# kubewharf/kubebrain

Measured on AMD Instinct MI355X. Metric: range+txn ops/s (90/10, Range limit=500) + watch events/s, higher is better.
Workload: dtype u8

## Files before the change

### kubebrain_amd/__init__.py

```python
from __future__ import annotations

import ctypes
import os

_HERE = os.path.dirname(os.path.abspath(__file__))
LIB_PATH = os.path.join(_HERE, "libkbslab.so")


def build(force: bool = False) -> str:
    import subprocess

    src_dir = os.path.join(_HERE, "csrc")
    srcs = [os.path.join(src_dir, f) for f in ("slab.hip", "store.cc", "cabi.cc",
                                               "comm.cc", "slab_dev.h", "store.h",
                                               "wpoll.h", "lplan.h", "gplan.h",
                                               "stepstage.h", "dmerge.h", "cplan.h")]
    srcs.append(os.path.join(_HERE, "..", "include", "kb_slab.h"))
    stale = force or not os.path.exists(LIB_PATH) or any(
        os.path.getmtime(s) > os.path.getmtime(LIB_PATH) for s in srcs)
    if stale:
        subprocess.check_call(["make", "-C", src_dir])
    return LIB_PATH


def load_library() -> ctypes.CDLL:
    if not os.path.exists(LIB_PATH):
        build()
    return ctypes.CDLL(LIB_PATH)


def open_store(store_prefix: bytes = b"/registry", **kw):
    from .client import Store

    if not os.path.exists(LIB_PATH):
        build()
    try:
        return Store(LIB_PATH, "kb_", store_prefix=store_prefix, **kw)
    except RuntimeError as e:
        lib = ctypes.CDLL(LIB_PATH)
        buf = ctypes.create_string_buffer(512)
        code = lib.kb_last_error(buf, 512)
        raise RuntimeError(
            f"kubebrain_amd: kb_new failed (status {code}): "
            f"{buf.value.decode(errors='replace')}") from e
```

### kubebrain_amd/csrc/slab.hip

```cpp

#include <hip/hip_runtime.h>

#include <chrono>
#include <cstdio>
#include <cstring>

#include "cplan.h"
#include "dmerge.h"
#include "slab_dev.h"
#include "stepstage.h"

namespace kbslab {

#define HIP_CHECK(expr)                                                    \
  do {                                                                     \
    hipError_t _e = (expr);                                                \
    if (_e != hipSuccess) {                                                \
      if (err) *err = std::string(#expr) + ": " + hipGetErrorString(_e);   \
      return false;                                                        \
    }                                                                      \
  } while (0)

#define HIP_CHECK_NULL(expr)                                               \
  do {                                                                     \
    hipError_t _e = (expr);                                                \
    if (_e != hipSuccess) {                                                \
      if (err) *err = std::string(#expr) + ": " + hipGetErrorString(_e);   \
      return nullptr;                                                      \
    }                                                                      \
  } while (0)

static inline int64_t ceil_div(int64_t a, int64_t b) { return (a + b - 1) / b; }


__device__ __forceinline__ int keycmp96(const uint8_t* a, const uint8_t* b) {
  const uint64_t* A = (const uint64_t*)a;
  const uint64_t* B = (const uint64_t*)b;
#pragma unroll
  for (int i = 0; i < KEYW / 8; ++i) {
    uint64_t x = A[i], y = B[i];
    if (x != y) {
      x = __builtin_bswap64(x);
      y = __builtin_bswap64(y);
      return x < y ? -1 : 1;
    }
  }
  return 0;
}

__device__ __forceinline__ int keycmp_ext(
    const uint8_t* a96, uint32_t alen, uint64_t ako, const uint8_t* aspill,
    const uint8_t* b96, uint32_t blen, uint64_t bko, const uint8_t* bspill) {
  int c = keycmp96(a96, b96);
  if (c || (alen <= (uint32_t)KEYW && blen <= (uint32_t)KEYW)) return c;
  uint32_t at = alen > (uint32_t)KEYW ? alen - KEYW : 0;
  uint32_t bt = blen > (uint32_t)KEYW ? blen - KEYW : 0;
  const uint8_t* ap = aspill + ako;
  const uint8_t* bp = bspill + bko;
  uint32_t m = at < bt ? at : bt;
  for (uint32_t i = 0; i < m; ++i)
    if (ap[i] != bp[i]) return ap[i] < bp[i] ? -1 : 1;
  return at == bt ? 0 : (at < bt ? -1 : 1);
}

struct Run {
  const uint8_t* keys;
  const uint64_t* meta;
  const uint64_t* rev;
  const uint64_t* vo;
  const uint64_t* ko;
};

struct QKey {
  const uint8_t* k96;
  uint32_t len;
  uint64_t ko;
  const uint8_t* tails;
};

__device__ __forceinline__ QKey row_qk(const Run& r, const uint8_t* spill,
                                       int64_t i) {
  return QKey{r.keys + i * KEYW, meta_klen(r.meta[i]), r.ko[i], spill};
}

__device__ __forceinline__ int rowcmp_q(const Run& r, const uint8_t* spill,
                                        int64_t i, const QKey& q) {
  return keycmp_ext(r.keys + i * KEYW, meta_klen(r.meta[i]), r.ko[i], spill,
                    q.k96, q.len, q.ko, q.tails);
}

__device__ int64_t d_lb_range(const Run& r, const uint8_t* spill, int64_t lo,
                              int64_t hi, const QKey& q, uint64_t qrev) {
  while (lo < hi) {
    int64_t mid = (lo + hi) >> 1;
    int c = rowcmp_q(r, spill, mid, q);
    if (c < 0 || (c == 0 && r.rev[mid] < qrev)) lo = mid + 1; else hi = mid;
  }
  return lo;
}

__device__ int64_t d_lb_wave(const Run& r, const uint8_t* spill, int64_t n,
                             const QKey& q, uint64_t qrev) {
  const int lane = threadIdx.x & 63;
  int64_t lo = 0, hi = n;
  while (hi - lo > 64) {
    int64_t step = (hi - lo) >> 6;
    int64_t p = lo + (int64_t)(lane + 1) * step;
    bool lt = false;
    if (p < hi) {
      int c = rowcmp_q(r, spill, p, q);
      lt = c < 0 || (c == 0 && r.rev[p] < qrev);
    }
    int k = __popcll(__ballot(lt));
    int64_t nlo = lo + (int64_t)k * step;
    int64_t nhi = k == 64 ? hi : min(lo + (int64_t)(k + 1) * step, hi);
    lo = nlo;
    hi = nhi;
  }
  int64_t p = lo + lane;
  bool ge = false;
  if (p < hi) {
    int c = rowcmp_q(r, spill, p, q);
    ge = !(c < 0 || (c == 0 && r.rev[p] < qrev));
  }
  uint64_t b = __ballot(ge);
  return b ? lo + (__ffsll((unsigned long long)b) - 1) : hi;
}

template <typename T>
__device__ __forceinline__ T block_excl_scan(T v, T* wsum, T* total) {
  const int lane = threadIdx.x & 63, w = threadIdx.x >> 6;
  const int nw = blockDim.x >> 6;
  T inc = v;
#pragma unroll
  for (int off = 1; off < 64; off <<= 1) {
    T o = __shfl_up(inc, off);
    if (lane >= off) inc += o;
  }
  if (lane == 63) wsum[w] = inc;
  __syncthreads();
  T base = 0, tot = 0;
  for (int i = 0; i < nw; ++i) {
    T s = wsum[i];
    if (i < w) base += s;
    tot += s;
  }
  __syncthreads();
  *total = tot;
  return base + inc - v;
}

__device__ __forceinline__ bool rows_same_key(const uint8_t* keys,
                                              const uint64_t* meta,
                                              const uint64_t* ko,
                                              const uint8_t* spill, int64_t i,
                                              int64_t j) {
  const uint64_t* a = (const uint64_t*)(keys + i * KEYW);
  const uint64_t* b = (const uint64_t*)(keys + j * KEYW);
#pragma unroll
  for (int k = 0; k < KEYW / 8; ++k)
    if (a[k] != b[k]) return false;
  uint32_t al = meta_klen(meta[i]), bl = meta_klen(meta[j]);
  if (al <= (uint32_t)KEYW && bl <= (uint32_t)KEYW) return true;
  if (al != bl) return false;
  const uint8_t* ap = spill + ko[i];
  const uint8_t* bp = spill + ko[j];
  for (uint32_t t = 0; t < al - (uint32_t)KEYW; ++t)
    if (ap[t] != bp[t]) return false;
  return true;
}

__global__ void k_same_next(const uint8_t* __restrict__ keys,
                            uint64_t* __restrict__ meta,
                            const uint64_t* __restrict__ ko,
                            const uint8_t* __restrict__ spill, int64_t n) {
  int64_t i = (int64_t)blockIdx.x * blockDim.x + threadIdx.x;
  if (i >= n) return;
// ... 90 lines not shown
        uint64_t sh = shadow ? shadow[i] : UINT64_MAX;
        if (rv > 0 && rv <= R && !(m & M_TOMB) &&
            !(sh != UINT64_MAX && sh <= R))
          win = !(m & M_SAME_NEXT) || rvn > R;
      }
      if (win) flags |= 1ull << r;
    }
    if (dbg0) { unsigned long long t1 = wall_clock64(); atomicAdd(&dbg[1], t1 - tprev); tprev = t1; }
    uint32_t wcnt = 0;
    for (int r = 0; r < rounds; ++r)
      wcnt += (uint32_t)__popcll(__ballot((flags >> r) & 1));
    if (dbg0) { unsigned long long t2 = wall_clock64(); atomicAdd(&dbg[2], t2 - tprev); tprev = t2; }
    if (lane == 0) wave_cnt[w] = (int)wcnt;
    __syncthreads();
    int64_t waveoff = 0, tile_total = 0;
    for (int k = 0; k < NW; ++k) {
      if (k < w) waveoff += wave_cnt[k];
      tile_total += wave_cnt[k];
    }
    if (out && wcnt) {
      uint32_t done = 0;
      for (int r = 0; r < rounds; ++r) {
        uint64_t b = __ballot((flags >> r) & 1);
        if ((flags >> r) & 1) {
          int64_t idx = cnt + waveoff + done +
                        (int64_t)__popcll(b & ((1ull << lane) - 1));
          if (idx < cap && idx < out_cap)
            out[idx] = (uint64_t)(wbase + ((int64_t)r << 6) + lane) | tagbit;
        }
        done += (uint32_t)__popcll(b);
      }
    }
    if (dbg0) { unsigned long long t3 = wall_clock64(); atomicAdd(&dbg[3], t3 - tprev); tprev = t3; }
    cnt += tile_total;
    scanned += min(TILE, hi - t);
    if (cnt >= cap) break;
    __syncthreads();
  }
  *total_out = cnt;
  if (scanned_accum) *scanned_accum += scanned;
  int64_t written = cnt < cap ? cnt : cap;
  if (written > out_cap) written = out_cap;
  return out ? written : 0;
}

__device__ int64_t d_lb_winlist(const uint64_t* rows, int64_t n, const Run& b,
                                const Run& d, const uint8_t* spill,
                                const QKey& q) {
  int64_t lo = 0, hi = n;
  while (lo < hi) {
    int64_t mid = (lo + hi) >> 1;
    uint64_t rt = rows[mid];
    const Run& rr = (rt & ROW_TAG_DELTA) ? d : b;
    if (rowcmp_q(rr, spill, (int64_t)(rt & ROW_MASK), q) < 0) lo = mid + 1;
    else hi = mid;
  }
  return lo;
}

__global__ void k_range_bounds(Run b, int64_t n, Run d, int64_t dn,
                               const uint8_t* __restrict__ spill,
                               const uint8_t* __restrict__ qtails,
                               const DevRangeQ* __restrict__ qs, int nq,
                               int64_t* __restrict__ bounds_g ,
                               unsigned long long* __restrict__ counters) {
  int q = blockIdx.x;
  if (q >= nq) return;
  if (q == 0 && threadIdx.x == 0) { counters[0] = 0; counters[1] = 0; }
  const DevRangeQ& Q = qs[q];
  const QKey qstart{Q.start, Q.start_klen, Q.start_ko, qtails};
  const QKey qend{Q.end, Q.end_klen, Q.end_ko, qtails};
  int w = threadIdx.x >> 6;
  int64_t r = -1;
  if (w == 0) r = d_lb_wave(b, spill, n, qstart, Q.start_rev);
  else if (w == 1) r = d_lb_wave(b, spill, n, qend, 0);
  else if (w == 2) r = d_lb_wave(d, spill, dn, qstart, Q.start_rev);
  else if (w == 3) r = d_lb_wave(d, spill, dn, qend, 0);
  if (w < 4 && (threadIdx.x & 63) == 0) bounds_g[(int64_t)q * 4 + w] = r;
}

__global__ void k_range_scan2(
    Run b, int64_t n, Run d, int64_t dn, const uint8_t* __restrict__ spill,
    const uint8_t* __restrict__ qtails, const DevRangeQ* __restrict__ qs,
    int nq, int64_t max_cap,
    uint64_t* __restrict__ rows_b, uint64_t* __restrict__ rows_d,
    uint64_t* __restrict__ rows_m, int64_t* __restrict__ found_out,
    int64_t* __restrict__ total_out, unsigned long long* __restrict__ scanned_out,
    const int64_t* __restrict__ bounds_g,
    const uint64_t* __restrict__ shadow,
    unsigned long long* dbg) {
  int q = blockIdx.x;
  if (q >= nq) return;
  __shared__ int wave_cnt[SCAN_T_MAX / 64];
  const DevRangeQ& Q = qs[q];
  const bool dbg0 = dbg && threadIdx.x == 0;
  unsigned long long tk0 = dbg0 ? wall_clock64() : 0;
  const int64_t lo_s = bounds_g[(int64_t)q * 4 + 0];
  const int64_t hi_s = bounds_g[(int64_t)q * 4 + 1];
  const int64_t dlo_s = bounds_g[(int64_t)q * 4 + 2];
  const int64_t dhi_s = bounds_g[(int64_t)q * 4 + 3];
  if (dbg0) { unsigned long long tkb = wall_clock64(); atomicAdd(&dbg[0], tkb - tk0); }
  const int64_t cap = Q.cap > 0 ? Q.cap : INT64_MAX;
  int64_t scanned = 0;
  int64_t dtotal = 0, btotal = 0;
  uint64_t* outd = Q.count_only ? nullptr : rows_d + (int64_t)q * max_cap;
  uint64_t* outb = Q.count_only ? nullptr : rows_b + (int64_t)q * max_cap;
  int64_t nB = scan_run_winners(d, spill, dlo_s, dhi_s, Q.read_rev,
                                cap, outd, max_cap, ROW_TAG_DELTA, nullptr,
                                &dtotal, &scanned, wave_cnt, dbg);
  __syncthreads();
  int64_t nA = scan_run_winners(b, spill, lo_s, hi_s, Q.read_rev, cap,
                                outb, max_cap, 0, dn ? shadow : nullptr,
                                &btotal, &scanned, wave_cnt, dbg);
  __syncthreads();
  unsigned long long tkm = dbg0 ? wall_clock64() : 0;
  int64_t cap_m = nA + nB;
  if (cap_m > cap) cap_m = cap;
  if (cap_m > max_cap) cap_m = max_cap;
  if (!Q.count_only) {
    uint64_t* outm = rows_m + (int64_t)q * max_cap;
    for (int64_t j = threadIdx.x; j < nA + nB; j += blockDim.x) {
      uint64_t rt;
      int64_t pos;
      if (j < nA) {
        rt = outb[j];
        QKey k = row_qk(b, spill, (int64_t)(rt & ROW_MASK));
        pos = j + d_lb_winlist(outd, nB, b, d, spill, k);
      } else {
        rt = outd[j - nA];
        QKey k = row_qk(d, spill, (int64_t)(rt & ROW_MASK));
        pos = (j - nA) + d_lb_winlist(outb, nA, b, d, spill, k);
      }
      if (pos < cap_m) outm[pos] = rt;
    }
  }
  if (dbg0) {
    unsigned long long tke = wall_clock64();
    atomicAdd(&dbg[4], tke - tkm);
    atomicAdd(&dbg[5], tke - tk0);
    atomicMax(&dbg[6], tke - tk0);
    atomicAdd(&dbg[7], 1ull);
  }
  if (threadIdx.x == 0) {
    total_out[q] = btotal + dtotal;
    found_out[q] = Q.count_only ? 0 : cap_m;
    atomicAdd(scanned_out, (unsigned long long)scanned);
  }
}

__global__ void k_get2(Run b, Run d, int64_t n, int64_t dn,
                       const uint8_t* __restrict__ spill,
                       const uint8_t* __restrict__ qtails,
                       const uint8_t* __restrict__ heap,
                       const DevGetQ* __restrict__ qs, int nq, int copy_vals,
                       uint8_t* __restrict__ out, int64_t slot,
                       uint64_t* __restrict__ orev, uint64_t* __restrict__ ometa,
                       int32_t* __restrict__ ofound, int32_t* __restrict__ oovf) {
  int q = blockIdx.x * (blockDim.x / 64) + (threadIdx.x >> 6);
  int lane = threadIdx.x & 63;
  if (q >= nq) return;
  const DevGetQ& Q = qs[q];
  const QKey qk{Q.key, Q.klen, Q.ko, qtails};
  int64_t row = -1;
  int isdelta = 0;
  uint64_t nr = Q.read_rev == UINT64_MAX ? UINT64_MAX : Q.read_rev + 1;
  if (dn > 0) {
    int64_t ub = d_lb_wave(d, spill, dn, qk, nr);
    if (ub > 0) {
      int64_t c = ub - 1;
      if (d.rev[c] >= 1 && rowcmp_q(d, spill, c, qk) == 0) {
        row = c;
        isdelta = 1;
      }
    }
  }
  if (row < 0) {
    int64_t ub = d_lb_wave(b, spill, n, qk, nr);
    if (ub > 0) {
      int64_t c = ub - 1;
      if (b.rev[c] >= 1 && rowcmp_q(b, spill, c, qk) == 0) row = c;
    }
  }
  if (row < 0) {
    if (lane == 0) { ofound[q] = 0; oovf[q] = 0; }
    return;
  }
  const uint64_t* meta = isdelta ? d.meta : b.meta;
  const uint64_t* rev = isdelta ? d.rev : b.rev;
  const uint64_t* vo = isdelta ? d.vo : b.vo;
  uint64_t m = meta[row];
  uint32_t vlen = meta_vlen(m);
  if (lane == 0) {
    ofound[q] = 1;
    orev[q] = rev[row];
    ometa[q] = m;
    oovf[q] = (copy_vals && vlen > slot) ? 1 : 0;
  }
  if (!copy_vals || vlen > slot) return;
  const uint8_t* vs = heap + vo[row];
  uint8_t* vd = out + (int64_t)q * slot;
  uint32_t w16 = vlen >> 4;
  for (uint32_t b = lane; b < w16; b += 64)
    ((uint4*)vd)[b] = ((const uint4*)vs)[b];
  if (lane == 0)
    for (uint32_t b = w16 * 16; b < vlen; ++b) vd[b] = vs[b];
}

__device__ __forceinline__ int64_t rec_bytes(uint32_t klen, uint32_t vlen) {
  return 16 + ((klen + 15) & ~15u) + ((vlen + 15) & ~15u);
}

__global__ void k_gather(Run b, Run d,
                         const uint8_t* __restrict__ heap,
                         const uint64_t* __restrict__ rows_out, int64_t max_cap,
                         const int64_t* __restrict__ found_out,
                         const DevRangeQ* __restrict__ qs, int nq,
                         uint8_t* __restrict__ gbuf, int64_t qcap,
                         int64_t* __restrict__ offs,
                         int64_t* __restrict__ gbytes_out,
                         int32_t* __restrict__ overflow,
                         unsigned long long* __restrict__ bytes_out) {
  int q = blockIdx.x;
  if (q >= nq) return;
  int64_t nwin = found_out[q];
  const bool konly = qs[q].keys_only != 0;
  const uint64_t* rows = rows_out + (int64_t)q * max_cap;
  int64_t* qoffs = offs + (int64_t)q * max_cap;
  __shared__ int64_t lds[256];
  __shared__ int64_t base_s;
  if (threadIdx.x == 0) base_s = 0;
  __syncthreads();
  for (int64_t c0 = 0; c0 < nwin; c0 += blockDim.x) {
    int64_t j = c0 + threadIdx.x;
// ... 253 lines not shown
                       const int32_t* __restrict__ overflow,
                       uint8_t* __restrict__ out, int nq) {
  int q = blockIdx.x;
  if (q >= nq) return;
  if (overflow[q]) return;
  int64_t bytes = gbytes[q];
  const uint4* src = (const uint4*)(gbuf + (int64_t)q * qcap);
  uint4* dst = (uint4*)(out + goffs[q]);
  int64_t words = bytes / 16;
  for (int64_t w = threadIdx.x; w < words; w += blockDim.x) dst[w] = src[w];
}

__global__ void k_block_scan(const uint64_t* __restrict__ in,
                             uint64_t* __restrict__ out,
                             uint64_t* __restrict__ sums, int64_t n) {
  __shared__ uint64_t lds[256];
  int64_t base = (int64_t)blockIdx.x * 256;
  int t = threadIdx.x;
  uint64_t v = base + t < n ? in[base + t] : 0;
  lds[t] = v;
  __syncthreads();
  for (int off = 1; off < 256; off <<= 1) {
    uint64_t add = t >= off ? lds[t - off] : 0;
    __syncthreads();
    lds[t] += add;
    __syncthreads();
  }
  if (base + t < n) out[base + t] = lds[t] - v;
  if (t == 255) sums[blockIdx.x] = lds[255];
}

__global__ void k_add_offsets(uint64_t* __restrict__ out,
                              const uint64_t* __restrict__ block_offs, int64_t n) {
  int64_t i = (int64_t)blockIdx.x * 256 + threadIdx.x;
  if (i < n) out[i] += block_offs[blockIdx.x];
}

__global__ void k_merge_newn(const uint64_t* __restrict__ dropx, int64_t n,
                             int64_t m, int64_t* __restrict__ out_n) {
  if (threadIdx.x == 0 && blockIdx.x == 0) *out_n = n - (int64_t)dropx[n] + m;
}

__global__ void k_fill_u64(uint64_t* a, uint64_t v, int64_t n) {
  int64_t i = (int64_t)blockIdx.x * blockDim.x + threadIdx.x;
  if (i < n) a[i] = v;
}

__global__ void k_find_bounds(Run a, int64_t n, const uint8_t* spill,
                              const uint8_t* bkeys, const uint64_t* brevs, int nb,
                              int64_t* out) {
  int i = blockIdx.x * blockDim.x + threadIdx.x;
  if (i < nb)
    out[i] = d_lb_range(a, spill, 0, n,
                        QKey{bkeys + (int64_t)i * KEYW, (uint32_t)KEYW, 0, nullptr},
                        brevs[i]);
}

__global__ void k_compact_mark(const uint64_t* __restrict__ meta,
                               const uint64_t* __restrict__ rev,
                               const uint64_t* __restrict__ vo, int64_t lo,
                               int64_t hi, uint64_t compact_rev,
                               uint64_t timeout_rev, uint64_t* __restrict__ keep) {
  int64_t i = lo + (int64_t)blockIdx.x * blockDim.x + threadIdx.x;
  if (i >= hi) return;
  uint64_t r = rev[i], m = meta[i];
  if (timeout_rev != 0 && (m & M_EVENTS)) {
    if (r == 0) {
      if (vo[i] <= timeout_rev) { keep[i] = 0; return; }
    } else if (r <= timeout_rev) { keep[i] = 0; return; }
  }
  if (r > compact_rev) return;
  if (r == 0) {
    if ((m & M_FLAG9) && vo[i] <= compact_rev) keep[i] = 0;
    return;
  }
  if (m & M_TOMB) { keep[i] = 0; return; }
  if ((m & M_SAME_NEXT) && rev[i + 1] <= compact_rev) keep[i] = 0;
}

__global__ void k_heap_sizes(const uint64_t* __restrict__ keep,
                             const uint64_t* __restrict__ rev,
                             const uint64_t* __restrict__ meta,
                             uint64_t* __restrict__ sz, int64_t n) {
  int64_t i = (int64_t)blockIdx.x * blockDim.x + threadIdx.x;
  if (i >= n) return;
  sz[i] = (keep[i] && rev[i] > 0) ? ((meta_vlen(meta[i]) + 15) & ~15ull) : 0;
}

__global__ void k_compact_scatter(const uint8_t* __restrict__ keysA,
                                  const uint64_t* __restrict__ metaA,
                                  const uint64_t* __restrict__ revA,
                                  const uint64_t* __restrict__ voA,
                                  const uint64_t* __restrict__ koA,
                                  const uint64_t* __restrict__ keep,
                                  const uint64_t* __restrict__ nidx,
                                  const uint64_t* __restrict__ heap_off,
                                  const uint64_t* __restrict__ spill_off,
                                  uint8_t* __restrict__ keysB,
                                  uint64_t* __restrict__ metaB,
                                  uint64_t* __restrict__ revB,
                                  uint64_t* __restrict__ voB,
                                  uint64_t* __restrict__ koB, int64_t n) {
  int64_t i = (int64_t)blockIdx.x * blockDim.x + threadIdx.x;
  if (i >= n || !keep[i]) return;
  int64_t j = (int64_t)nidx[i];
  revB[j] = revA[i];
  metaB[j] = metaA[i];
// ... 5 lines not shown
  for (int k = 0; k < KEYW / 8; ++k) kd[k] = ks[k];
}

__global__ void k_spill_sizes(const uint64_t* __restrict__ keep,
                              const uint64_t* __restrict__ meta,
                              uint64_t* __restrict__ sz, int64_t n) {
  int64_t i = (int64_t)blockIdx.x * blockDim.x + threadIdx.x;
  if (i >= n) return;
  uint32_t kl = meta_klen(meta[i]);
  sz[i] = (keep[i] && kl > (uint32_t)KEYW) ? (((uint64_t)kl - KEYW + 15) & ~15ull) : 0;
}

__global__ void k_spill_scatter(const uint64_t* __restrict__ keep,
                                const uint64_t* __restrict__ meta,
                                const uint64_t* __restrict__ koA,
                                const uint64_t* __restrict__ spill_off,
                                const uint8_t* __restrict__ spillA,
                                uint8_t* __restrict__ spillB, int64_t n) {
  int64_t i = (int64_t)blockIdx.x * (blockDim.x / 64) + (threadIdx.x >> 6);
  int lane = threadIdx.x & 63;
  if (i >= n || !keep[i]) return;
  uint32_t kl = meta_klen(meta[i]);
  if (kl <= (uint32_t)KEYW) return;
  uint32_t t = kl - (uint32_t)KEYW;
  const uint8_t* src = spillA + koA[i];
  uint8_t* dst = spillB + spill_off[i];
  for (uint32_t x = lane; x < t; x += 64) dst[x] = src[x];
}

__global__ void k_heap_scatter(const uint64_t* __restrict__ keep,
                               const uint64_t* __restrict__ rev,
                               const uint64_t* __restrict__ meta,
                               const uint64_t* __restrict__ voA,
                               const uint64_t* __restrict__ heap_off,
                               const uint8_t* __restrict__ heapA,
                               uint8_t* __restrict__ heapB, int64_t n) {
  int64_t i = (int64_t)blockIdx.x * (blockDim.x / 64) + (threadIdx.x >> 6);
  int lane = threadIdx.x & 63;
  if (i >= n || !keep[i] || rev[i] == 0) return;
  uint64_t bytes = (meta_vlen(meta[i]) + 15) & ~15ull;
  const uint4* src = (const uint4*)(heapA + voA[i]);
  uint4* dst = (uint4*)(heapB + heap_off[i]);
  for (uint64_t w = lane; w < bytes / 16; w += 64) dst[w] = src[w];
}

__global__ __launch_bounds__(256) void k_delta_rank(
    Run a, int64_t n, Run dnew, int64_t m, const uint8_t* __restrict__ spill,
    int64_t* __restrict__ lbs , uint32_t* __restrict__ dups ) {
  const int64_t j = (int64_t)blockIdx.x * 4 + (threadIdx.x >> 6);
  if (j >= m) return;
  QKey k = row_qk(dnew, spill, j);
  const uint64_t rv = dnew.rev[j];
  const int64_t lb = d_lb_wave(a, spill, n, k, rv);
  const bool dup = lb < n && a.rev[lb] == rv && rowcmp_q(a, spill, lb, k) == 0;
  if ((threadIdx.x & 63) == 0) {
    lbs[j] = lb;
    dups[j] = dup ? 1 : 0;
  }
}

__device__ __forceinline__ void copy_row(const Run& s, int64_t i,
                                         uint8_t* keysB, uint64_t* metaB,
                                         uint64_t* revB, uint64_t* voB,
                                         uint64_t* koB, int64_t out) {
  revB[out] = s.rev[i];
  metaB[out] = s.meta[i];
  voB[out] = s.vo[i];
  koB[out] = s.ko[i];
  const uint4* ks = (const uint4*)(s.keys + i * KEYW);
  uint4* kd = (uint4*)(keysB + out * KEYW);
#pragma unroll
  for (int t = 0; t < KEYW / 16; ++t) kd[t] = ks[t];
}

__global__ __launch_bounds__(256) void k_delta_scatter(
    Run a, int64_t n, Run dnew, int64_t m,
    const int64_t* __restrict__ lbs, const uint32_t* __restrict__ dups,
    uint64_t* __restrict__ outpos ,
    uint8_t* keysB, uint64_t* metaB, uint64_t* revB, uint64_t* voB,
    uint64_t* koB, int64_t* __restrict__ newn_out) {
  __shared__ int64_t s_lb[kbmerge::kMaxNew];
  __shared__ uint16_t s_dupx[kbmerge::kMaxNew + 4];
  __shared__ uint32_t s_ws[4];
  const int t = threadIdx.x, mi = (int)m;
  for (int x = t; x < mi; x += 256) s_lb[x] = lbs[x];
  uint32_t d[4], sum = 0;
#pragma unroll
  for (int u = 0; u < 4; ++u) {
    d[u] = 4 * t + u < mi ? dups[4 * t + u] : 0;
    sum += d[u];
  }
  uint32_t tot;
  uint32_t run = block_excl_scan<uint32_t>(sum, s_ws, &tot);
#pragma unroll
  for (int u = 0; u < 4; ++u) {
    if (4 * t + u < mi) s_dupx[4 * t + u] = (uint16_t)run;
    run += d[u];
  }
  if (t == 0) s_dupx[mi] = (uint16_t)tot;
  __syncthreads();
  const int64_t g = (int64_t)blockIdx.x * 256 + t;
  if (g < n) {
    const int64_t out = kbmerge::OldSlot(g, s_lb, s_dupx, mi);
    if (out >= 0) copy_row(a, g, keysB, metaB, revB, voB, koB, out);
  } else if (g < n + m) {
    const int j = (int)(g - n);
    const int64_t out = kbmerge::NewSlot(j, s_lb, s_dupx);
    outpos[j] = (uint64_t)out;
    copy_row(dnew, j, keysB, metaB, revB, voB, koB, out);
  }
  if (g == 0) *newn_out = kbmerge::NewCount(n, mi, s_dupx);
}

__global__ void k_merge_rank_inv_big(Run a, int64_t n, Run dnew, int64_t m,
                                     const uint8_t* __restrict__ spill,
                                     uint64_t* __restrict__ v ,
                                     uint64_t* __restrict__ drop ,
                                     uint64_t* __restrict__ dup ,
                                     uint64_t* __restrict__ lbs ) {
  int64_t j = (int64_t)blockIdx.x * blockDim.x + threadIdx.x;
  if (j >= m) return;
  QKey k = row_qk(dnew, spill, j);
  int64_t lb = d_lb_range(a, spill, 0, n, k, dnew.rev[j]);
  bool isdup = lb < n && a.rev[lb] == dnew.rev[j] &&
               rowcmp_q(a, spill, lb, k) == 0;
  lbs[j] = (uint64_t)lb;
  if (isdup) {
    dup[j] = 1;
    drop[lb] = 1;
    atomicAdd(&v[lb + 1], (uint64_t)-1ll);
  }
  atomicAdd(&v[lb + (isdup ? 1 : 0)], 1ull);
}

__global__ void k_merge_scatter_delta2(
    Run dnew, int64_t m, const uint64_t* __restrict__ dupx ,
    uint64_t* __restrict__ lbs, uint8_t* keysB, uint64_t* metaB,
    uint64_t* revB, uint64_t* voB, uint64_t* koB) {
  int64_t j = (int64_t)blockIdx.x * blockDim.x + threadIdx.x;
  if (j >= m) return;
  int64_t out = (int64_t)lbs[j] + j - (int64_t)dupx[j];
  lbs[j] = (uint64_t)out;
  revB[out] = dnew.rev[j];
  metaB[out] = dnew.meta[j];
  voB[out] = dnew.vo[j];
  koB[out] = dnew.ko[j];
  const uint4* ks = (const uint4*)(dnew.keys + j * KEYW);
  uint4* kd = (uint4*)(keysB + out * KEYW);
#pragma unroll
  for (int t = 0; t < KEYW / 16; ++t) kd[t] = ks[t];
}

__global__ void k_set_newn(const uint64_t* __restrict__ dupx, int64_t n,
                           int64_t m, int64_t* __restrict__ newn_out) {
  if (threadIdx.x == 0 && blockIdx.x == 0)
    *newn_out = n + m - (int64_t)dupx[m];
}

__global__ void k_merge_scatter_base2(
    Run a, const uint64_t* __restrict__ sv ,
    const uint64_t* __restrict__ drop, uint8_t* keysB, uint64_t* metaB,
    uint64_t* revB, uint64_t* voB, uint64_t* koB, int64_t n) {
  int64_t i = (int64_t)blockIdx.x * blockDim.x + threadIdx.x;
  if (i >= n || drop[i]) return;
  int64_t j = i + (int64_t)sv[i + 1];
  revB[j] = a.rev[i];
  metaB[j] = a.meta[i];
  voB[j] = a.vo[i];
  koB[j] = a.ko[i];
  const uint4* ks = (const uint4*)(a.keys + i * KEYW);
  uint4* kd = (uint4*)(keysB + j * KEYW);
#pragma unroll
  for (int t = 0; t < KEYW / 16; ++t) kd[t] = ks[t];
}

__global__ void k_same_next_fixup(uint8_t* __restrict__ keys,
                                  uint64_t* __restrict__ meta,
                                  const uint64_t* __restrict__ ko,
                                  const uint8_t* __restrict__ spill,
                                  int64_t new_n,
                                  const uint64_t* __restrict__ outpos,
                                  int64_t m) {
  int64_t t = (int64_t)blockIdx.x * blockDim.x + threadIdx.x;
  if (t >= 2 * m) return;
  int64_t i = (int64_t)outpos[t >> 1] - (t & 1);
  if (i < 0 || i >= new_n) return;
  uint64_t mm = meta[i];
  bool same = i + 1 < new_n && rows_same_key(keys, meta, ko, spill, i, i + 1);
  meta[i] = same ? (mm | M_SAME_NEXT) : (mm & ~M_SAME_NEXT);
}

__global__ void k_merge_scatter_delta(
    Run a, int64_t n, Run dnew, int64_t m, const uint8_t* __restrict__ spill,
    const uint64_t* __restrict__ dropx,
    uint8_t* keysB, uint64_t* metaB, uint64_t* revB, uint64_t* voB,
    uint64_t* koB) {
  int64_t j = (int64_t)blockIdx.x * blockDim.x + threadIdx.x;
  if (j >= m) return;
  QKey k = row_qk(dnew, spill, j);
  int64_t lb = d_lb_range(a, spill, 0, n, k, dnew.rev[j]);
  int64_t out = lb - (int64_t)dropx[lb] + j;
  revB[out] = dnew.rev[j];
  metaB[out] = dnew.meta[j];
  voB[out] = dnew.vo[j];
  koB[out] = dnew.ko[j];
  const uint64_t* ks = (const uint64_t*)(dnew.keys + j * KEYW);
  uint64_t* kd = (uint64_t*)(keysB + out * KEYW);
#pragma unroll
  for (int kk = 0; kk < KEYW / 8; ++kk) kd[kk] = ks[kk];
}

__global__ void k_merge_small(Run src, int64_t n, Run dnew, int64_t m,
                              const uint8_t* __restrict__ spill,
                              uint8_t* __restrict__ okeys,
                              uint64_t* __restrict__ ometa,
                              uint64_t* __restrict__ orev,
                              uint64_t* __restrict__ ovo,
                              uint64_t* __restrict__ oko,
                              int64_t* __restrict__ out_n) {
  __shared__ uint16_t dropx[8193];
  __shared__ uint16_t partial[257];
  int t = threadIdx.x;
  const int T = blockDim.x;
  int chunk = (int)((n + T - 1) / T);
  int i0 = t * chunk;
  int i1 = min((int64_t)i0 + chunk, n);
  uint16_t cnt = 0;
  for (int i = i0; i < i1; ++i) {
    QKey k = row_qk(src, spill, i);
    int64_t lb = d_lb_range(dnew, spill, 0, m, k, src.rev[i]);
    bool drop = lb < m && dnew.rev[lb] == src.rev[i] &&
                rowcmp_q(dnew, spill, lb, k) == 0;
    dropx[i] = drop ? 1 : 0;
    cnt += drop;
  }
  partial[t] = cnt;
  __syncthreads();
  if (t == 0) {
    uint16_t acc = 0;
    for (int k = 0; k < T; ++k) { uint16_t v = partial[k]; partial[k] = acc; acc += v; }
    partial[T] = acc;
  }
  __syncthreads();
  {
    uint16_t acc = partial[t];
    for (int i = i0; i < i1; ++i) { uint16_t v = dropx[i]; dropx[i] = acc; acc += v; }
  }
  __syncthreads();
  int64_t dropped = partial[T];
  int64_t new_n = n - dropped + m;
  if (t == 0) *out_n = new_n;
  for (int64_t i = t; i < n; i += T) {
    QKey k = row_qk(src, spill, i);
    int64_t lb = d_lb_range(dnew, spill, 0, m, k, src.rev[i]);
    bool drop = lb < m && dnew.rev[lb] == src.rev[i] &&
                rowcmp_q(dnew, spill, lb, k) == 0;
    if (drop) continue;
    int64_t j = i - (int64_t)dropx[i] + lb;
    orev[j] = src.rev[i];
    ometa[j] = src.meta[i];
    ovo[j] = src.vo[i];
    oko[j] = src.ko[i];
    const uint64_t* ks = (const uint64_t*)(src.keys + i * KEYW);
    uint64_t* kd = (uint64_t*)(okeys + j * KEYW);
#pragma unroll
    for (int k2 = 0; k2 < KEYW / 8; ++k2) kd[k2] = ks[k2];
  }
  for (int64_t j = t; j < m; j += T) {
    QKey k = row_qk(dnew, spill, j);
    int64_t lb = d_lb_range(src, spill, 0, n, k, dnew.rev[j]);
    int64_t dpx = lb < n ? dropx[lb] : (int64_t)dropped;
    int64_t o = lb - dpx + j;
    orev[o] = dnew.rev[j];
    ometa[o] = dnew.meta[j];
    ovo[o] = dnew.vo[j];
    oko[o] = dnew.ko[j];
    const uint64_t* ks = (const uint64_t*)(dnew.keys + j * KEYW);
    uint64_t* kd = (uint64_t*)(okeys + o * KEYW);
#pragma unroll
    for (int k2 = 0; k2 < KEYW / 8; ++k2) kd[k2] = ks[k2];
  }
  __syncthreads();
  for (int64_t i = t; i < new_n; i += T) {
    bool same = i + 1 < new_n &&
                rows_same_key(okeys, ometa, oko, spill, i, i + 1);
    ometa[i] = same ? (ometa[i] | M_SAME_NEXT) : (ometa[i] & ~M_SAME_NEXT);
  }
}


__global__ void k_watch_filter2(const uint8_t* __restrict__ er_keys,
                                const uint64_t* __restrict__ er_rev,
                                int64_t ring_cap, int64_t base_seq,
                                int64_t count,
                                const uint8_t* __restrict__ wpfx,
                                const uint32_t* __restrict__ wplen,
                                const uint64_t* __restrict__ wfrom,
                                const uint32_t* __restrict__ wlive, int64_t W,
                                uint64_t* __restrict__ bitmap, int64_t words) {
  __shared__ uint64_t lkeys[64 * (KEYW / 8)];
  __shared__ uint64_t lrev[64];
  const int64_t w = (int64_t)blockIdx.x * 64 + threadIdx.x;
  const int64_t c0 = (int64_t)blockIdx.y << 6;
  const int64_t cn = min((int64_t)64, count - c0);
  for (int64_t v = threadIdx.x; v < cn * (KEYW / 8); v += 64) {
    int64_t j = v / (KEYW / 8), k = v % (KEYW / 8);
    int64_t slot = (base_seq + c0 + j) % ring_cap;
    lkeys[v] = ((const uint64_t*)(er_keys + slot * KEYW))[k];
  }
  if (threadIdx.x < cn) {
// ... 248 lines not shown
  if (g >= cum[nq]) return;
  int lo = 0, hi = nq;
  while (hi - lo > 1) {
    const int mid = (lo + hi) >> 1;
    if (cum[mid] <= g) lo = mid; else hi = mid;
  }
  const int q = lo;
  const uint64_t j = g - cum[q];
  if (j >= (uint64_t)max_cap) return;
  const uint64_t rt = rows_m[(int64_t)q * max_cap + (int64_t)j];
  const bool isd = (rt & ROW_TAG_DELTA) != 0;
  const int64_t row = (int64_t)(rt & ROW_MASK);
  if (row >= (isd ? dn : n)) return;
  const Run& r = isd ? rd : rb;
  const uint64_t m = r.meta[row];
  const uint32_t klen = meta_klen(m);
  const uint32_t vlen = qs[q].keys_only ? 0 : meta_vlen(m);
  const uint64_t dd = sec_base[q] + offs[(int64_t)q * max_cap + (int64_t)j];
  const uint64_t reclen = 16 + (uint64_t)klen + vlen;
  if (dd > (uint64_t)arena_cap || reclen > (uint64_t)arena_cap - dd) return;
  uint8_t* dst = arena + dd;
  const uint64_t rev = r.rev[row];
  if (lane < 8) dst[lane] = (uint8_t)(rev >> (8 * lane));
  else if (lane < 12) dst[lane] = (uint8_t)(klen >> (8 * (lane - 8)));
  else if (lane < 16) dst[klen + lane] = (uint8_t)(vlen >> (8 * (lane - 12)));
  const uint32_t kin = klen > (uint32_t)KEYW ? (uint32_t)KEYW : klen;
  wp_copy_record(r.keys + row * KEYW, dst + 12, kin, lane);
  if (klen > (uint32_t)KEYW) {
    const uint64_t ko = r.ko[row];
    const uint32_t tl = klen - (uint32_t)KEYW;
    if ((ko & 15) == 0 && ko + ((tl + 15) & ~15u) <= (uint64_t)spill_used)
      wp_copy_record(spill + ko, dst + 12 + KEYW, tl, lane);
  }
  if (vlen) {
    const uint64_t vo = r.vo[row];
    if ((vo & 15) == 0 &&
        vo + (((uint64_t)vlen + 15) & ~15ull) <= (uint64_t)heap_used)
      wp_copy_record(heap + vo, dst + 16 + klen, vlen, lane);
  }
}


constexpr uint64_t GET_ROW_NONE = ~0ull;

__global__ __launch_bounds__(256) void k_get_find(
    Run b, Run d, int64_t n, int64_t dn, const uint8_t* __restrict__ spill,
    const uint8_t* __restrict__ qtails, const DevGetQ* __restrict__ qs, int nq,
    uint64_t* __restrict__ otag, uint64_t* __restrict__ orev,
    uint64_t* __restrict__ ometa) {
  const int q = blockIdx.x * 4 + (threadIdx.x >> 6);
  const int lane = threadIdx.x & 63;
  if (q >= nq) return;
  const DevGetQ& Q = qs[q];
  const QKey qk{Q.key, Q.klen, Q.ko, qtails};
  const uint64_t nr = Q.read_rev == UINT64_MAX ? UINT64_MAX : Q.read_rev + 1;
  uint64_t tag = GET_ROW_NONE;
  if (dn > 0) {
    const int64_t ub = d_lb_wave(d, spill, dn, qk, nr);
    if (ub > 0 && d.rev[ub - 1] >= 1 && rowcmp_q(d, spill, ub - 1, qk) == 0)
      tag = ROW_TAG_DELTA | (uint64_t)(ub - 1);
  }
  if (tag == GET_ROW_NONE) {
    const int64_t ub = d_lb_wave(b, spill, n, qk, nr);
    if (ub > 0 && b.rev[ub - 1] >= 1 && rowcmp_q(b, spill, ub - 1, qk) == 0)
      tag = (uint64_t)(ub - 1);
  }
  if (lane != 0) return;
  otag[q] = tag;
  if (tag == GET_ROW_NONE) {
    orev[q] = 0;
    ometa[q] = 0;
  } else {
    const Run& r = (tag & ROW_TAG_DELTA) ? d : b;
    const int64_t row = (int64_t)(tag & ROW_MASK);
    orev[q] = r.rev[row];
    ometa[q] = r.meta[row];
  }
}

__global__ __launch_bounds__(256) void k_get_plan(
    const uint64_t* __restrict__ tag, const uint64_t* __restrict__ rev,
    const uint64_t* __restrict__ meta, int nq, int no_values,
    uint64_t committed, uint64_t* __restrict__ aoff,
    uint64_t* __restrict__ hdr) {
  const int lane = threadIdx.x & 63, w = threadIdx.x >> 6;
  __shared__ uint64_t wsum[4];
  uint64_t base = 0;
  for (int c0 = 0; c0 < nq; c0 += 256) {
    const int q = c0 + threadIdx.x;
    uint64_t vlen = 0, mod = 0;
    bool has = false;
    if (q < nq) {
      const uint64_t m = meta[q];
      has = tag[q] != GET_ROW_NONE && !(m & M_TOMB);
      if (has) {
        mod = rev[q];
        vlen = no_values ? 0 : meta_vlen(m);
      }
    }
    const uint64_t incl = wp_scan64(vlen, lane);
    if (lane == 63) wsum[w] = incl;
    __syncthreads();
    uint64_t woff = 0, tot = 0;
#pragma unroll
    for (int k = 0; k < 4; ++k) {
      if (k < w) woff += wsum[k];
      tot += wsum[k];
    }
    if (q < nq) {
      aoff[q] = base + woff + incl - vlen;
      uint64_t* e = hdr + 2 + 4 * (int64_t)q;
      e[0] = (uint64_t)(has ? 1 : 0) << 32;
      e[1] = mod > committed ? mod : committed;
      e[2] = mod;
      e[3] = vlen;
    }
    base += tot;
    __syncthreads();
// ... 2318 lines not shown
```

Baseline: 2.395 million.

## Replace early-exit key compare with branchless wide-load comparator and cache merge bounds

Adds a shared key-compare header that loads a full 96-byte key row with 16-byte vector loads, preloads meta/ko/rev in one batch, and compares branchlessly by picking the first differing word. Binary searches and merge duplicate checks now fold the revision tiebreak into a single ordered compare. The shared-memory merge also caches each row's lower bound from its first pass, so the scatter pass skips the second binary search. This trades reading all 96 bytes for every compare (no early exit), plus extra shared memory, for fewer divergent branches and wider memory transactions in latency-bound searches.

```diff
diff --git a/kubebrain_amd/__init__.py b/kubebrain_amd/__init__.py
--- a/kubebrain_amd/__init__.py
+++ b/kubebrain_amd/__init__.py
@@ -14,7 +14,8 @@
     srcs = [os.path.join(src_dir, f) for f in ("slab.hip", "store.cc", "cabi.cc",
                                                "comm.cc", "slab_dev.h", "store.h",
                                                "wpoll.h", "lplan.h", "gplan.h",
-                                               "stepstage.h", "dmerge.h", "cplan.h")]
+                                               "stepstage.h", "dmerge.h", "cplan.h",
+                                               "keycmp.h")]
     srcs.append(os.path.join(_HERE, "..", "include", "kb_slab.h"))
     stale = force or not os.path.exists(LIB_PATH) or any(
         os.path.getmtime(s) > os.path.getmtime(LIB_PATH) for s in srcs)
diff --git a/kubebrain_amd/csrc/keycmp.h b/kubebrain_amd/csrc/keycmp.h
--- /dev/null
+++ b/kubebrain_amd/csrc/keycmp.h
@@ -0,0 +1,109 @@
+#pragma once
+
+#include <cstdint>
+#include <cstring>
+
+#ifdef __HIPCC__
+#define KBK_HD __host__ __device__
+#define KBK_UNROLL _Pragma("unroll")
+#else
+#define KBK_HD
+#define KBK_UNROLL
+#endif
+
+namespace kbkey {
+
+constexpr int kKeyW = 96;
+constexpr int kWords = kKeyW / 8;
+
+struct Key96 {
+  uint64_t w[kWords];
+};
+
+template <int kAlign>
+KBK_HD inline Key96 Load96(const uint8_t* p) {
+  Key96 k;
+  KBK_UNROLL
+  for (int t = 0; t < kKeyW / kAlign; ++t)
+    memcpy((uint8_t*)k.w + t * kAlign,
+           __builtin_assume_aligned(p + t * kAlign, kAlign), kAlign);
+  return k;
+}
+
+KBK_HD inline int Cmp96(const Key96& a, const Key96& b) {
+  uint64_t x = 0, y = 0;
+  KBK_UNROLL
+  for (int i = kWords - 1; i >= 0; --i) {
+    const bool ne = a.w[i] != b.w[i];
+    x = ne ? a.w[i] : x;
+    y = ne ? b.w[i] : y;
+  }
+  x = __builtin_bswap64(x);
+  y = __builtin_bswap64(y);
+  return x < y ? -1 : (x > y ? 1 : 0);
+}
+
+KBK_HD inline bool Eq96(const Key96& a, const Key96& b) {
+  uint64_t d = 0;
+  KBK_UNROLL
+  for (int i = 0; i < kWords; ++i) d |= a.w[i] ^ b.w[i];
+  return d == 0;
+}
+
+KBK_HD inline int CmpTails(const uint8_t* at, uint32_t alen, const uint8_t* bt,
+                           uint32_t blen) {
+  const uint32_t an = alen > (uint32_t)kKeyW ? alen - kKeyW : 0;
+  const uint32_t bn = blen > (uint32_t)kKeyW ? blen - kKeyW : 0;
+  const uint32_t m = an < bn ? an : bn;
+  for (uint32_t i = 0; i < m; ++i)
+    if (at[i] != bt[i]) return at[i] < bt[i] ? -1 : 1;
+  return an == bn ? 0 : (an < bn ? -1 : 1);
+}
+
+struct KeyR {
+  Key96 k;
+  uint32_t len;
+  uint64_t ko;
+  const uint8_t* tails;
+};
+
+KBK_HD inline int CmpKeys(const KeyR& a, const KeyR& b) {
+  const int c = Cmp96(a.k, b.k);
+  if (c != 0 || (a.len <= (uint32_t)kKeyW && b.len <= (uint32_t)kKeyW))
+    return c;
+  return CmpTails(a.tails + a.ko, a.len, b.tails + b.ko, b.len);
+}
+
+struct Probe {
+  KeyR key;
+  uint64_t rev;
+};
+
+KBK_HD inline Probe LoadProbe(const uint8_t* keys, const uint64_t* meta,
+                              const uint64_t* ko, const uint64_t* rev,
+                              const uint8_t* spill, int64_t i) {
+  Probe p;
+  p.key.k = Load96<16>(keys + i * kKeyW);
+  uint64_t m = meta[i];
+  p.key.ko = ko[i];
+  p.rev = rev[i];
+#ifdef __HIP_DEVICE_COMPILE__
+  asm volatile(""
+               : "+v"(p.key.k.w[0]), "+v"(p.key.k.w[1]), "+v"(p.key.k.w[2]),
+                 "+v"(p.key.k.w[3]), "+v"(p.key.k.w[4]), "+v"(p.key.k.w[5]),
+                 "+v"(p.key.k.w[6]), "+v"(p.key.k.w[7]), "+v"(p.key.k.w[8]),
+                 "+v"(p.key.k.w[9]), "+v"(p.key.k.w[10]), "+v"(p.key.k.w[11]),
+                 "+v"(m), "+v"(p.key.ko), "+v"(p.rev));
+#endif
+  p.key.len = (uint32_t)((m >> 16) & 0xffff);
+  p.key.tails = spill;
+  return p;
+}
+
+KBK_HD inline int Order(const Probe& p, const KeyR& q, uint64_t qrev) {
+  const int c = CmpKeys(p.key, q);
+  const int r = p.rev < qrev ? -1 : (p.rev > qrev ? 1 : 0);
+  return c != 0 ? c : r;
+}
+
+}
diff --git a/kubebrain_amd/csrc/keycmp_hostcheck.cc b/kubebrain_amd/csrc/keycmp_hostcheck.cc
--- /dev/null
+++ b/kubebrain_amd/csrc/keycmp_hostcheck.cc
@@ -0,0 +1,156 @@
+#include <cstdio>
+#include <cstdlib>
+#include <cstring>
+#include <string>
+#include <vector>
+
+#include "keycmp.h"
+
+#define CHECK(c)                                                      \
+  do {                                                                \
+    if (!(c)) {                                                       \
+      fprintf(stderr, "%s:%d: check failed: %s\n", __FILE__, __LINE__, #c); \
+      return 1;                                                       \
+    }                                                                 \
+  } while (0)
+
+using namespace kbkey;
+
+static int sgn(int x) { return x < 0 ? -1 : (x > 0 ? 1 : 0); }
+
+static int ref_keycmp(const std::string& a, const std::string& b) {
+  const size_t m = a.size() < b.size() ? a.size() : b.size();
+  const int c = m ? sgn(memcmp(a.data(), b.data(), m)) : 0;
+  if (c) return c;
+  return a.size() == b.size() ? 0 : (a.size() < b.size() ? -1 : 1);
+}
+
+struct Row {
+  std::string key;
+  uint64_t rev;
+};
+
+struct Cols {
+  uint8_t* keys = nullptr;
+  uint64_t *meta = nullptr, *ko = nullptr, *rev = nullptr;
+  uint8_t* spill = nullptr;
+  size_t n = 0;
+  explicit Cols(const std::vector<Row>& rows) : n(rows.size()) {
+    keys = (uint8_t*)aligned_alloc(16, n * kKeyW);
+    memset(keys, 0, n * kKeyW);
+    meta = (uint64_t*)malloc(n * 8);
+    ko = (uint64_t*)malloc(n * 8);
+    rev = (uint64_t*)malloc(n * 8);
+    size_t tails = 0;
+    for (const Row& r : rows)
+      if (r.key.size() > (size_t)kKeyW) tails += r.key.size() - kKeyW;
+    spill = (uint8_t*)malloc(tails ? tails : 1);
+    size_t off = 0;
+    for (size_t i = 0; i < n; ++i) {
+      const std::string& k = rows[i].key;
+      const size_t head = k.size() < (size_t)kKeyW ? k.size() : (size_t)kKeyW;
+      memcpy(keys + i * kKeyW, k.data(), head);
+      meta[i] = ((uint64_t)(k.size() & 0xffff) << 16) | 0xfull |
+                ((uint64_t)0x1234 << 32);
+      ko[i] = 0;
+      if (k.size() > (size_t)kKeyW) {
+        ko[i] = off;
+        memcpy(spill + off, k.data() + kKeyW, k.size() - kKeyW);
+        off += k.size() - kKeyW;
+      }
+      rev[i] = rows[i].rev;
+    }
+  }
+  ~Cols() {
+    free(keys); free(meta); free(ko); free(rev); free(spill);
+  }
+  Cols(const Cols&) = delete;
+  Cols& operator=(const Cols&) = delete;
+};
+
+static int check_all_pairs(const std::vector<Row>& rows, long* pairs) {
+  Cols c(rows);
+  for (size_t i = 0; i < rows.size(); ++i) {
+    const Probe p = LoadProbe(c.keys, c.meta, c.ko, c.rev, c.spill, (int64_t)i);
+    CHECK(p.key.len == rows[i].key.size());
+    CHECK(p.rev == rows[i].rev);
+    for (size_t j = 0; j < rows.size(); ++j) {
+      KeyR q;
+      q.k = Load96<8>(c.keys + j * kKeyW);
+      q.len = (uint32_t)rows[j].key.size();
+      q.ko = c.ko[j];
+      q.tails = c.spill;
+      const int kc = ref_keycmp(rows[i].key, rows[j].key);
+      CHECK(CmpKeys(p.key, q) == kc);
+      CHECK(Eq96(p.key.k, q.k) ==
+            (memcmp(c.keys + i * kKeyW, c.keys + j * kKeyW, kKeyW) == 0));
+      CHECK(Cmp96(p.key.k, q.k) ==
+            sgn(memcmp(c.keys + i * kKeyW, c.keys + j * kKeyW, kKeyW)));
+      const uint64_t qrevs[] = {0, rows[i].rev - 1, rows[i].rev,
+                                rows[i].rev + 1, rows[j].rev, UINT64_MAX};
+      for (uint64_t qrev : qrevs) {
+        const int want =
+            kc ? kc : (rows[i].rev < qrev ? -1 : (rows[i].rev > qrev ? 1 : 0));
+        CHECK(Order(p, q, qrev) == want);
+      }
+      ++*pairs;
+    }
+  }
+  return 0;
+}
+
+int main() {
+  long pairs = 0;
+  std::vector<Row> rows;
+  const std::string base(96, 'm');
+  rows.push_back({base, 5});
+  for (int w = 0; w < kWords; ++w)
+    for (int b : {0, 7})
+      for (char ch : {'a', 'z', '\x7f', '\xff'}) {
+        std::string k = base;
+        k[8 * w + b] = ch;
+        rows.push_back({k, 5});
+        rows.push_back({k.substr(0, 8 * w + b + 1), 6});
+      }
+  if (check_all_pairs(rows, &pairs)) return 1;
+
+  rows.clear();
+  const std::string p96(96, 'k');
+  rows.push_back({p96, 7});
+  rows.push_back({p96, 9});
+  rows.push_back({p96 + "a", 7});
+  rows.push_back({p96 + "a", 8});
+  rows.push_back({p96 + "b", 7});
+  const std::string t203(203, 'q');
+  rows.push_back({p96 + "a" + t203, 7});
+  rows.push_back({p96 + "a" + t203, 3});
+  { std::string k = p96 + "a" + t203; k[97] = 'r'; rows.push_back({k, 7}); }
+  { std::string k = p96 + "a" + t203; k[200] = 'p'; rows.push_back({k, 7}); }
+  { std::string k = p96 + "a" + t203; k[299] = 'r'; rows.push_back({k, 7}); }
+  rows.push_back({(p96 + "a" + t203).substr(0, 299), 7});
+  rows.push_back({p96.substr(0, 95), 7});
+  rows.push_back({std::string(96, 'k').replace(95, 1, "j"), 7});
+  rows.push_back({"k", 1});
+  rows.push_back({"kk", 1});
+  rows.push_back({"/registry/pods/ns-0001/pod-000001", 4});
+  rows.push_back({"/registry/pods/ns-0001/pod-000001", 1000000});
+  rows.push_back({"/registry/pods/ns-0001/pod-000002", 4});
+  rows.push_back({"/registry/pods/ns-0002/pod-000001", 4});
+  if (check_all_pairs(rows, &pairs)) return 1;
+
+  uint64_t s = 0x9e3779b97f4a7c15ull;
+  auto rnd = [&]() { s ^= s << 13; s ^= s >> 7; s ^= s << 17; return s; };
+  for (int round = 0; round < 20; ++round) {
+    rows.clear();
+    for (int i = 0; i < 40; ++i) {
+      const size_t lens[] = {1, 33, 95, 96, 97, 130, 300};
+      std::string k(lens[rnd() % 7], 'x');
+      for (size_t t = k.size() > 3 ? k.size() - 3 : 0; t < k.size(); ++t)
+        k[t] = (rnd() & 1) ? 'x' : 'y';
+      rows.push_back({k, 1 + rnd() % 3});
+    }
+    if (check_all_pairs(rows, &pairs)) return 1;
+  }
+  printf("keycmp hostcheck OK: %ld ordered pairs\n", pairs);
+  return 0;
+}
diff --git a/kubebrain_amd/csrc/slab.hip b/kubebrain_amd/csrc/slab.hip
--- a/kubebrain_amd/csrc/slab.hip
+++ b/kubebrain_amd/csrc/slab.hip
@@ -7,6 +7,7 @@
 
 #include "cplan.h"
 #include "dmerge.h"
+#include "keycmp.h"
 #include "slab_dev.h"
 #include "stepstage.h"
 
@@ -33,36 +34,6 @@
 static inline int64_t ceil_div(int64_t a, int64_t b) { return (a + b - 1) / b; }
 
 
-__device__ __forceinline__ int keycmp96(const uint8_t* a, const uint8_t* b) {
-  const uint64_t* A = (const uint64_t*)a;
-  const uint64_t* B = (const uint64_t*)b;
-#pragma unroll
-  for (int i = 0; i < KEYW / 8; ++i) {
-    uint64_t x = A[i], y = B[i];
-    if (x != y) {
-      x = __builtin_bswap64(x);
-      y = __builtin_bswap64(y);
-      return x < y ? -1 : 1;
-    }
-  }
-  return 0;
-}
-
-__device__ __forceinline__ int keycmp_ext(
-    const uint8_t* a96, uint32_t alen, uint64_t ako, const uint8_t* aspill,
-    const uint8_t* b96, uint32_t blen, uint64_t bko, const uint8_t* bspill) {
-  int c = keycmp96(a96, b96);
-  if (c || (alen <= (uint32_t)KEYW && blen <= (uint32_t)KEYW)) return c;
-  uint32_t at = alen > (uint32_t)KEYW ? alen - KEYW : 0;
-  uint32_t bt = blen > (uint32_t)KEYW ? blen - KEYW : 0;
-  const uint8_t* ap = aspill + ako;
-  const uint8_t* bp = bspill + bko;
-  uint32_t m = at < bt ? at : bt;
-  for (uint32_t i = 0; i < m; ++i)
-    if (ap[i] != bp[i]) return ap[i] < bp[i] ? -1 : 1;
-  return at == bt ? 0 : (at < bt ? -1 : 1);
-}
-
 struct Run {
   const uint8_t* keys;
   const uint64_t* meta;
@@ -71,30 +42,42 @@
   const uint64_t* ko;
 };
 
-struct QKey {
-  const uint8_t* k96;
-  uint32_t len;
-  uint64_t ko;
-  const uint8_t* tails;
-};
+
+using QKey = kbkey::KeyR;
+static_assert(kbkey::kKeyW == KEYW, "key column width");
+
+__device__ __forceinline__ QKey load_qk(const uint8_t* k96, uint32_t len,
+                                        uint64_t ko, const uint8_t* tails) {
+  return QKey{kbkey::Load96<8>(k96), len, ko, tails};
+}
+
+__device__ __forceinline__ kbkey::Probe row_probe(const Run& r,
+                                                  const uint8_t* spill,
+                                                  int64_t i) {
+  return kbkey::LoadProbe(r.keys, r.meta, r.ko, r.rev, spill, i);
+}
 
 __device__ __forceinline__ QKey row_qk(const Run& r, const uint8_t* spill,
                                        int64_t i) {
-  return QKey{r.keys + i * KEYW, meta_klen(r.meta[i]), r.ko[i], spill};
+  return row_probe(r, spill, i).key;
 }
 
 __device__ __forceinline__ int rowcmp_q(const Run& r, const uint8_t* spill,
                                         int64_t i, const QKey& q) {
-  return keycmp_ext(r.keys + i * KEYW, meta_klen(r.meta[i]), r.ko[i], spill,
-                    q.k96, q.len, q.ko, q.tails);
+  return kbkey::CmpKeys(row_probe(r, spill, i).key, q);
+}
+
+__device__ __forceinline__ int rowcmp_q(const Run& r, const uint8_t* spill,
+                                        int64_t i, const QKey& q,
+                                        uint64_t qrev) {
+  return kbkey::Order(row_probe(r, spill, i), q, qrev);
 }
 
 __device__ int64_t d_lb_range(const Run& r, const uint8_t* spill, int64_t lo,
                               int64_t hi, const QKey& q, uint64_t qrev) {
   while (lo < hi) {
     int64_t mid = (lo + hi) >> 1;
-    int c = rowcmp_q(r, spill, mid, q);
-    if (c < 0 || (c == 0 && r.rev[mid] < qrev)) lo = mid + 1; else hi = mid;
+    if (rowcmp_q(r, spill, mid, q, qrev) < 0) lo = mid + 1; else hi = mid;
   }
   return lo;
 }
@@ -107,10 +90,7 @@
     int64_t step = (hi - lo) >> 6;
     int64_t p = lo + (int64_t)(lane + 1) * step;
     bool lt = false;
-    if (p < hi) {
-      int c = rowcmp_q(r, spill, p, q);
-      lt = c < 0 || (c == 0 && r.rev[p] < qrev);
-    }
+    if (p < hi) lt = rowcmp_q(r, spill, p, q, qrev) < 0;
     int k = __popcll(__ballot(lt));
     int64_t nlo = lo + (int64_t)k * step;
     int64_t nhi = k == 64 ? hi : min(lo + (int64_t)(k + 1) * step, hi);
@@ -119,10 +99,7 @@
   }
   int64_t p = lo + lane;
   bool ge = false;
-  if (p < hi) {
-    int c = rowcmp_q(r, spill, p, q);
-    ge = !(c < 0 || (c == 0 && r.rev[p] < qrev));
-  }
+  if (p < hi) ge = rowcmp_q(r, spill, p, q, qrev) >= 0;
   uint64_t b = __ballot(ge);
   return b ? lo + (__ffsll((unsigned long long)b) - 1) : hi;
 }
@@ -319,7 +296,7 @@
     int64_t mid = (lo + hi) >> 1;
     uint64_t rt = rows[mid];
     const Run& rr = (rt & ROW_TAG_DELTA) ? d : b;
-    if (rowcmp_q(rr, spill, (int64_t)(rt & ROW_MASK), q) < 0) lo = mid + 1;
+    if (rowcmp_q(rr, spill, (int64_t)(rt & ROW_MASK), q, 0) < 0) lo = mid + 1;
     else hi = mid;
   }
   return lo;
@@ -335,14 +312,17 @@
   if (q >= nq) return;
   if (q == 0 && threadIdx.x == 0) { counters[0] = 0; counters[1] = 0; }
   const DevRangeQ& Q = qs[q];
-  const QKey qstart{Q.start, Q.start_klen, Q.start_ko, qtails};
-  const QKey qend{Q.end, Q.end_klen, Q.end_ko, qtails};
   int w = threadIdx.x >> 6;
   int64_t r = -1;
-  if (w == 0) r = d_lb_wave(b, spill, n, qstart, Q.start_rev);
-  else if (w == 1) r = d_lb_wave(b, spill, n, qend, 0);
-  else if (w == 2) r = d_lb_wave(d, spill, dn, qstart, Q.start_rev);
-  else if (w == 3) r = d_lb_wave(d, spill, dn, qend, 0);
+  if (w < 4) {
+    const bool is_end = w & 1;
+    const QKey qk = load_qk(is_end ? Q.end : Q.start,
+                            is_end ? Q.end_klen : Q.start_klen,
+                            is_end ? Q.end_ko : Q.start_ko, qtails);
+    const uint64_t qrev = is_end ? 0 : Q.start_rev;
+    r = w < 2 ? d_lb_wave(b, spill, n, qk, qrev)
+              : d_lb_wave(d, spill, dn, qk, qrev);
+  }
   if (w < 4 && (threadIdx.x & 63) == 0) bounds_g[(int64_t)q * 4 + w] = r;
 }
 
@@ -427,7 +407,7 @@
   int lane = threadIdx.x & 63;
   if (q >= nq) return;
   const DevGetQ& Q = qs[q];
-  const QKey qk{Q.key, Q.klen, Q.ko, qtails};
+  const QKey qk = load_qk(Q.key, Q.klen, Q.ko, qtails);
   int64_t row = -1;
   int isdelta = 0;
   uint64_t nr = Q.read_rev == UINT64_MAX ? UINT64_MAX : Q.read_rev + 1;
@@ -435,7 +415,8 @@
     int64_t ub = d_lb_wave(d, spill, dn, qk, nr);
     if (ub > 0) {
       int64_t c = ub - 1;
-      if (d.rev[c] >= 1 && rowcmp_q(d, spill, c, qk) == 0) {
+      const kbkey::Probe pr = row_probe(d, spill, c);
+      if (pr.rev >= 1 && kbkey::CmpKeys(pr.key, qk) == 0) {
         row = c;
         isdelta = 1;
       }
@@ -445,7 +426,8 @@
     int64_t ub = d_lb_wave(b, spill, n, qk, nr);
     if (ub > 0) {
       int64_t c = ub - 1;
-      if (b.rev[c] >= 1 && rowcmp_q(b, spill, c, qk) == 0) row = c;
+      const kbkey::Probe pr = row_probe(b, spill, c);
+      if (pr.rev >= 1 && kbkey::CmpKeys(pr.key, qk) == 0) row = c;
     }
   }
   if (row < 0) {
@@ -805,7 +787,7 @@
   int i = blockIdx.x * blockDim.x + threadIdx.x;
   if (i < nb)
     out[i] = d_lb_range(a, spill, 0, n,
-                        QKey{bkeys + (int64_t)i * KEYW, (uint32_t)KEYW, 0, nullptr},
+                        load_qk(bkeys + (int64_t)i * KEYW, (uint32_t)KEYW, 0, nullptr),
                         brevs[i]);
 }
 
@@ -917,7 +899,7 @@
   QKey k = row_qk(dnew, spill, j);
   const uint64_t rv = dnew.rev[j];
   const int64_t lb = d_lb_wave(a, spill, n, k, rv);
-  const bool dup = lb < n && a.rev[lb] == rv && rowcmp_q(a, spill, lb, k) == 0;
+  const bool dup = lb < n && rowcmp_q(a, spill, lb, k, rv) == 0;
   if ((threadIdx.x & 63) == 0) {
     lbs[j] = lb;
     dups[j] = dup ? 1 : 0;
@@ -987,8 +969,7 @@
   if (j >= m) return;
   QKey k = row_qk(dnew, spill, j);
   int64_t lb = d_lb_range(a, spill, 0, n, k, dnew.rev[j]);
-  bool isdup = lb < n && a.rev[lb] == dnew.rev[j] &&
-               rowcmp_q(a, spill, lb, k) == 0;
+  bool isdup = lb < n && rowcmp_q(a, spill, lb, k, dnew.rev[j]) == 0;
   lbs[j] = (uint64_t)lb;
   if (isdup) {
     dup[j] = 1;
@@ -1084,6 +1065,7 @@
                               uint64_t* __restrict__ oko,
                               int64_t* __restrict__ out_n) {
   __shared__ uint16_t dropx[8193];
+  __shared__ uint16_t lbx[8192];
   __shared__ uint16_t partial[257];
   int t = threadIdx.x;
   const int T = blockDim.x;
@@ -1092,11 +1074,11 @@
   int i1 = min((int64_t)i0 + chunk, n);
   uint16_t cnt = 0;
   for (int i = i0; i < i1; ++i) {
-    QKey k = row_qk(src, spill, i);
-    int64_t lb = d_lb_range(dnew, spill, 0, m, k, src.rev[i]);
-    bool drop = lb < m && dnew.rev[lb] == src.rev[i] &&
-                rowcmp_q(dnew, spill, lb, k) == 0;
+    const kbkey::Probe pr = row_probe(src, spill, i);
+    int64_t lb = d_lb_range(dnew, spill, 0, m, pr.key, pr.rev);
+    bool drop = lb < m && rowcmp_q(dnew, spill, lb, pr.key, pr.rev) == 0;
     dropx[i] = drop ? 1 : 0;
+    lbx[i] = drop ? (uint16_t)0xffff : (uint16_t)lb;
     cnt += drop;
   }
   partial[t] = cnt;
@@ -1116,11 +1098,8 @@
   int64_t new_n = n - dropped + m;
   if (t == 0) *out_n = new_n;
   for (int64_t i = t; i < n; i += T) {
-    QKey k = row_qk(src, spill, i);
-    int64_t lb = d_lb_range(dnew, spill, 0, m, k, src.rev[i]);
-    bool drop = lb < m && dnew.rev[lb] == src.rev[i] &&
-                rowcmp_q(dnew, spill, lb, k) == 0;
-    if (drop) continue;
+    const uint16_t lb = lbx[i];
+    if (lb == 0xffff) continue;
     int64_t j = i - (int64_t)dropx[i] + lb;
     orev[j] = src.rev[i];
     ometa[j] = src.meta[i];
@@ -1475,18 +1454,24 @@
   const int lane = threadIdx.x & 63;
   if (q >= nq) return;
   const DevGetQ& Q = qs[q];
-  const QKey qk{Q.key, Q.klen, Q.ko, qtails};
+  const QKey qk = load_qk(Q.key, Q.klen, Q.ko, qtails);
   const uint64_t nr = Q.read_rev == UINT64_MAX ? UINT64_MAX : Q.read_rev + 1;
   uint64_t tag = GET_ROW_NONE;
   if (dn > 0) {
     const int64_t ub = d_lb_wave(d, spill, dn, qk, nr);
-    if (ub > 0 && d.rev[ub - 1] >= 1 && rowcmp_q(d, spill, ub - 1, qk) == 0)
-      tag = ROW_TAG_DELTA | (uint64_t)(ub - 1);
+    if (ub > 0) {
+      const kbkey::Probe pr = row_probe(d, spill, ub - 1);
+      if (pr.rev >= 1 && kbkey::CmpKeys(pr.key, qk) == 0)
+        tag = ROW_TAG_DELTA | (uint64_t)(ub - 1);
+    }
   }
   if (tag == GET_ROW_NONE) {
     const int64_t ub = d_lb_wave(b, spill, n, qk, nr);
-    if (ub > 0 && b.rev[ub - 1] >= 1 && rowcmp_q(b, spill, ub - 1, qk) == 0)
-      tag = (uint64_t)(ub - 1);
+    if (ub > 0) {
+      const kbkey::Probe pr = row_probe(b, spill, ub - 1);
+      if (pr.rev >= 1 && kbkey::CmpKeys(pr.key, qk) == 0)
+        tag = (uint64_t)(ub - 1);
+    }
   }
   if (lane != 0) return;
   otag[q] = tag;
```

Result: slower. 2.355 million (-1.7%).
